# ethan-li-coding/AD-Census

Measured on NVIDIA H100. Metric: disparity-maps/sec (450x375x64), higher is better.
Workload: dtype f32

## Files before the change

### adcensus_b200/csrc/k_scanline.cu

```cuda
#include "adc_common.cuh"
#include "so_plan.h"
#include <cuda.h>
#include <string.h>

template <int K>
struct Piece { static constexpr int G = (K % 4 == 0) ? 4 : ((K % 2 == 0) ? 2 : 1); static constexpr int NP = K / G; };

template <int K>
__device__ __forceinline__ void ld_vec(const float* p, int lane, int Dp, float (&v)[K]) {
    constexpr int G = Piece<K>::G, NP = Piece<K>::NP;
#pragma unroll
    for (int j = 0; j < NP; j++) {
        const int d = lane * K + j * G;
        if (d < Dp) {
            if (G == 4) { const float4 t = *reinterpret_cast<const float4*>(p + d); v[j*G] = t.x; v[j*G+1] = t.y; v[j*G+2] = t.z; v[j*G+3] = t.w; }
            else if (G == 2) { const float2 t = *reinterpret_cast<const float2*>(p + d); v[j*G] = t.x; v[j*G+1] = t.y; }
            else v[j] = p[d];
        } else {
#pragma unroll
            for (int g = 0; g < G; g++) v[j * G + g] = 0.f;
        }
    }
}

template <int K>
__device__ __forceinline__ void st_vec(float* __restrict__ p, int lane, int Dp, const float (&v)[K]) {
    constexpr int G = Piece<K>::G, NP = Piece<K>::NP;
#pragma unroll
    for (int j = 0; j < NP; j++) {
        const int d = lane * K + j * G;
        if (d < Dp) {
            if (G == 4) *reinterpret_cast<float4*>(p + d) = make_float4(v[j*G], v[j*G+1], v[j*G+2], v[j*G+3]);
            else if (G == 2) *reinterpret_cast<float2*>(p + d) = make_float2(v[j*G], v[j*G+1]);
            else p[d] = v[j];
        }
    }
}

__host__ __device__ inline int so_row_words(int W) { return (W + 31) / 32 + 2; }

__global__ void __launch_bounds__(128)
k_so_bitrows(AdcDims dm, int tso, const uint8_t* __restrict__ dmap, unsigned* __restrict__ bitrows) {
    const int pair = blockIdx.y, y = blockIdx.x;
    const int W = dm.W, rw = so_row_words(W);
    const uint8_t* mh = dmap + ((size_t)pair * 4 + 2) * dm.N;
    const uint8_t* mv = dmap + ((size_t)pair * 4 + 3) * dm.N;
    const int lane = threadIdx.x & 31, wid = threadIdx.x >> 5;
    unsigned* out = bitrows + (((size_t)pair * 4 + wid) * dm.H + y) * rw;
    for (int w0 = 0; w0 < rw; w0++) {
        const int j = w0 * 32 + lane;
        const int xr = W - 1 - j;
        bool bit = false;
        if (xr > 0 && xr < W - 1) {
            int v;
            if (wid == 0) v = mh[y * W + xr];
            else if (wid == 1) v = mh[y * W + xr + 1];
            else if (wid == 2) v = y > 0 ? mv[y * W + xr] : 255;
            else v = y + 1 < dm.H ? mv[(y + 1) * W + xr] : 255;
            bit = v < tso;
        }
        const unsigned m = __ballot_sync(0xffffffffu, bit);
        if (lane == 0) out[w0] = m;
    }
}

__global__ void __launch_bounds__(256)
k_so_records(AdcDims dm, int tso, const uint8_t* __restrict__ dmap,
             const unsigned* __restrict__ bitrows, unsigned* __restrict__ rec) {
    const int pair = blockIdx.y;
    const int i = blockIdx.x * blockDim.x + threadIdx.x;
    if (i >= dm.N) return;
    const int sx = blockIdx.z == 0 ? 1 : (blockIdx.z == 1 ? -1 : 0);
    const int sy = blockIdx.z == 2 ? 1 : (blockIdx.z == 3 ? -1 : 0);
    const int W = dm.W, D = dm.D, dmin = dm.dmin;
    const int y = i / W, x = i - y * W;
    const bool fwd = (sx + sy) > 0;
    const int pstep = sx + sy * W;
    const int variant = sx ? (fwd ? 0 : 1) : (fwd ? 2 : 3);
    const int rw = so_row_words(W), nrec = so_rec_words(dm.Dp);
    unsigned* out = rec + (((size_t)pair * 4 + variant) * dm.N + i) * nrec;
    const uint8_t* ml = dmap + ((size_t)pair * 4 + (sx ? 0 : 1)) * dm.N;
    const int pi_from = i - pstep;
    int d1 = 0;
    if (fwd) d1 = ml[i];
    else if (pi_from >= 0 && pi_from < dm.N) d1 = ml[pi_from];
    const unsigned a1 = d1 < tso ? 0xffffffffu : 0u;
    const int lo = max(0, x - dmin - (W - 2));
    const int hi = min(D - 1, x - dmin - 1);
    const unsigned* row = bitrows + (((size_t)pair * 4 + variant) * dm.H + y) * rw;
    const int j0 = W - 1 - x + dmin;
    auto window = [&](int d0) -> unsigned {
        const int j = j0 + d0;
        const int wlo = j >> 5;
        const int sh = j & 31;
        const unsigned a = (wlo >= 0 && wlo < rw) ? row[wlo] : 0u;
        const unsigned b = (wlo + 1 >= 0 && wlo + 1 < rw) ? row[wlo + 1] : 0u;
        return __funnelshift_r(a, b, sh);
    };
    unsigned fill_hi = a1;
    if (lo <= hi) fill_hi = (window(hi) & 1u) ? 0xffffffffu : 0u;
    const int nw = (dm.Dp + 31) / 32 + 1;
    auto word = [&](int w0) -> unsigned {
        if (lo > hi) return a1;
        const int d0 = w0 * 32;
        const unsigned raw = window(d0);
        const unsigned m_lo = lo <= d0 ? 0u : (lo >= d0 + 32 ? 0xffffffffu : ((1u << (lo - d0)) - 1u));
        const unsigned m_hi = hi >= d0 + 31 ? 0u : (hi < d0 ? 0xffffffffu : ~((2u << (hi - d0)) - 1u));
        return (raw & ~m_lo & ~m_hi) | (a1 & m_lo) | (fill_hi & m_hi);
    };
    if (nrec == 4) {
        *reinterpret_cast<uint4*>(out) = make_uint4(a1, word(0), nw > 1 ? word(1) : 0u, nw > 2 ? word(2) : 0u);
        return;
    }
    out[0] = a1;
    for (int w0 = 0; w0 < nw; w0++) out[1 + w0] = word(w0);
    for (int w0 = 1 + nw; w0 < nrec; w0++) out[w0] = 0u;
}

__device__ __forceinline__ unsigned so_smem_u32(const void* p) { return (unsigned)__cvta_generic_to_shared(p); }
__device__ __forceinline__ void mbar_init(unsigned bar, unsigned count) {
    asm volatile("mbarrier.init.shared::cta.b64 [%0], %1;" ::"r"(bar), "r"(count) : "memory");
}
__device__ __forceinline__ void mbar_expect_tx(unsigned bar, unsigned bytes) {
    asm volatile("mbarrier.arrive.expect_tx.shared::cta.b64 _, [%0], %1;" ::"r"(bar), "r"(bytes) : "memory");
}
__device__ __forceinline__ void mbar_wait(unsigned bar, unsigned parity) {
    unsigned ok, spins = 0;
    do {
        asm volatile("{\n\t.reg .pred p;\n\tmbarrier.try_wait.parity.shared::cta.b64 p, [%1], %2;\n\tselp.u32 %0, 1, 0, p;\n\t}"
                     : "=r"(ok) : "r"(bar), "r"(parity) : "memory");
        if (!ok && ++spins > (1u << 24)) __trap();
    } while (!ok);
}
__device__ __forceinline__ void tma_load_4d(unsigned dst, const CUtensorMap* map, int c0, int c1, int c2, int c3, unsigned bar) {
    asm volatile("cp.async.bulk.tensor.4d.shared::cluster.global.tile.mbarrier::complete_tx::bytes [%0], [%1, {%2, %3, %4, %5}], [%6];"
                 ::"r"(dst), "l"(reinterpret_cast<unsigned long long>(map)), "r"(c0), "r"(c1), "r"(c2), "r"(c3), "r"(bar)
                 : "memory");
}

template <int K, int LPS, bool FULL, bool WTA>
__device__ __forceinline__ void so_pass(const CUtensorMap& tm_cost, const CUtensorMap& tm_rec, const AdcParams& P,
                                        float* __restrict__ dst, float* __restrict__ disp_l, int sx, int sy, int T, int NS) {
    constexpr int LPW = 32 / LPS;
    if constexpr (WTA) { sx = 0; sy = -1; }
    extern __shared__ __align__(128) unsigned char so_smem[];
    const AdcDims& dm = P.dm;
    const int lane = threadIdx.x & 31, wid = threadIdx.x >> 5;
    const int sub = lane / LPS, gl = lane % LPS;
    const int line0 = (blockIdx.x * SO_WARPS + wid) * LPW;
    const int line = line0 + sub;
    const int pair = blockIdx.y;
    const int n_lines = sx ? dm.H : dm.W, n_steps = sx ? dm.W : dm.H;
    if (line0 >= n_lines) return;
    const bool live = line < n_lines;
    const int W = dm.W, D = FULL ? K * LPS : dm.D, Dp = FULL ? K * LPS : dm.Dp;
    const int pstep = sx + sy * W;
    const int nrec = so_rec_words(Dp);
    const bool fwd = sx + sy > 0;
    const int variant = sx ? (sx > 0 ? 0 : 1) : (sy > 0 ? 2 : 3);
    const unsigned cost_region = so_cost_region(Dp, T), slot_bytes = so_slot_bytes(Dp, T);
    unsigned char* wring = so_smem + (size_t)wid * NS * slot_bytes;
    const unsigned bar0 = so_smem_u32(so_smem + (size_t)SO_WARPS * NS * slot_bytes) + (unsigned)(wid * NS) * 8u;
    const unsigned tx = (unsigned)(T * LPW * (Dp + nrec) * 4);
    const int nch = (n_steps + T - 1) / T;

    auto issue = [&](int c) {
        const int s = c % NS;
        const unsigned bar = bar0 + 8u * (unsigned)s, d0 = so_smem_u32(wring + (size_t)s * slot_bytes);
        const int p0 = fwd ? c * T : n_steps - (c + 1) * T;
        mbar_expect_tx(bar, tx);
        if (sx) {
            tma_load_4d(d0, &tm_cost, 0, p0, line0, pair, bar);
            tma_load_4d(d0 + cost_region, &tm_rec, 0, p0, line0, pair * 4 + variant, bar);
        } else {
            tma_load_4d(d0, &tm_cost, 0, line0, p0, pair, bar);
            tma_load_4d(d0 + cost_region, &tm_rec, 0, line0, p0, pair * 4 + variant, bar);
        }
    };
    if (lane == 0) {
        for (int j = 0; j < NS; j++) mbar_init(bar0 + 8u * j, 1);
        asm volatile("fence.mbarrier_init.release.cluster;" ::: "memory");
        for (int c = 0; c < NS && c < nch; c++) issue(c);
    }
    __syncwarp();

    int c = 0, t = 0, slot = 0;
    unsigned phase = 0;
    const int bit0 = gl * K;
    auto fetch = [&](float (&C)[K], bool& a1, unsigned& bits) -> float* {
        if (t == 0) mbar_wait(bar0 + 8u * (unsigned)slot, phase);
        const int pos = fwd ? t : T - 1 - t;
        const int row = sx ? sub * T + pos : pos * LPW + sub;
        unsigned char* sl = wring + (size_t)slot * slot_bytes;
        float* cs = reinterpret_cast<float*>(sl) + row * Dp;
        if constexpr (FULL && K == 8) {
            const int b = (gl >> 2) & 1;
            const float4 u = *reinterpret_cast<const float4*>(cs + 8 * gl + 4 * b);
            const float4 v = *reinterpret_cast<const float4*>(cs + 8 * gl + 4 - 4 * b);
            const float4 lo = b ? v : u, hi = b ? u : v;
            C[0] = lo.x; C[1] = lo.y; C[2] = lo.z; C[3] = lo.w;
            C[4] = hi.x; C[5] = hi.y; C[6] = hi.z; C[7] = hi.w;
        } else ld_vec<K>(cs, gl, Dp, C);
        const unsigned* rw = reinterpret_cast<const unsigned*>(sl + cost_region) + row * nrec;
        a1 = rw[0] != 0u;
        bits = __funnelshift_r(rw[1 + (bit0 >> 5)], rw[2 + (bit0 >> 5)], bit0 & 31);
        if (!WTA && ++t == T) {
            asm volatile("fence.proxy.async.shared::cta;" ::: "memory");
            __syncwarp();
            if (lane == 0 && c + NS < nch) issue(c + NS);
            t = 0;
            c++;
            if (++slot == NS) { slot = 0; phase ^= 1u; }
        }
        return cs;
    };

    bool valid[K];
#pragma unroll
    for (int k = 0; k < K; k++) valid[k] = FULL || (gl * K + k) < D;

    const int wta_threads = 32 * min(SO_WARPS, (n_lines - (int)blockIdx.x * SO_WARPS * LPW + LPW - 1) / LPW);
    auto wta_left = [&](const float* row, const float (&V)[K], float m, int step) {
        int kk = K;
#pragma unroll
        for (int k = K - 1; k >= 0; k--)
            if (valid[k] && V[k] == m) kk = k;
        const unsigned bal = __ballot_sync(0xffffffffu, kk < K);
        const unsigned grp = LPS == 32 ? bal : (bal >> (sub * LPS)) & ((1u << LPS) - 1u);
        __syncwarp();
        if (live && gl == __ffs(grp) - 1) {
            const int bd = gl * K + kk;
            float out = ADC_INVALID_F;
            if (m < ADC_LARGE_F && bd > 0 && bd < D - 1) out = adc_subpixel(row[bd - 1], row[bd + 1], m, dm.dmin + bd);
            disp_l[(size_t)pair * dm.N + (size_t)(dm.H - 1 - step) * W + line] = out;
        }
    };
    auto wta_records = [&](int nt, int s0) {
        constexpr int CB = SO_WARPS * LPW;
        const int x0 = blockIdx.x * CB, NJ = CB + D - 1, nb = (W + CB - 1) / CB, dmin = dm.dmin;
        const long long plane = (long long)dm.H * nb * NJ;
        float* R = dst + (size_t)pair * dm.vol_stride;
        const size_t wstride = (size_t)NS * slot_bytes / 4;
        const int xcap = W - 1 - x0;
        for (int tt = 0; tt < nt; tt++) {
            const int y = dm.H - 1 - (s0 + tt);
            const float* rb = reinterpret_cast<const float*>(so_smem + (size_t)slot * slot_bytes) + (T - 1 - tt) * LPW * Dp;
            for (int j = threadIdx.x; j < NJ; j += wta_threads) {
                const int xr = x0 - dmin - (D - 1) + j;
                const int ilo = max(0, j - (D - 1)), ihi = min(min(CB - 1, j), xcap);
                if (xr < 0 || xr >= W || ilo > ihi) continue;
                const int dd0 = D - 1 - j;
                auto at = [&](int i) { return rb[(size_t)(i / LPW) * wstride + (i % LPW) * Dp + i + dd0]; };
                float m = ADC_LARGE_F;
                int a = -1;
                const float* pw = rb + dd0;
#pragma unroll 1
                for (int w = 0; w < SO_WARPS; w++, pw += wstride + LPW) {
                    const float* p = pw;
#pragma unroll
                    for (int s = 0; s < LPW; s++, p += Dp + 1) {
                        const int i = w * LPW + s;
                        if (i >= ilo && i <= ihi) {
                            const float v = *p;
                            if (m > v) { m = v; a = i; }
                        }
                    }
                }
                const long long r = ((long long)y * nb + blockIdx.x) * NJ + j;
                R[r] = m;
                R[plane + r] = __int_as_float(a < 0 ? -1 : a + dd0);
                R[2 * plane + r] = a > ilo ? at(a - 1) : ADC_LARGE_F;
                R[3 * plane + r] = a >= 0 && a < ihi ? at(a + 1) : ADC_LARGE_F;
                R[4 * plane + r] = at(ilo);
                R[5 * plane + r] = at(ihi);
            }
        }
    };
    auto wta_advance = [&](int step) {
        if (++t < T && step + 1 < n_steps) return;
        asm volatile("bar.sync 1, %0;" ::"r"(wta_threads) : "memory");
        wta_records(t, step + 1 - t);
        asm volatile("fence.proxy.async.shared::cta;" ::: "memory");
        asm volatile("bar.sync 1, %0;" ::"r"(wta_threads) : "memory");
        if (lane == 0 && c + NS < nch) issue(c + NS);
        t = 0;
        c++;
        if (++slot == NS) { slot = 0; phase ^= 1u; }
    };

    long long pi = (long long)(sy ? (sy > 0 ? 0 : dm.H - 1) : line) * W + (sx ? (sx > 0 ? 0 : W - 1) : line);
    float* O = dst + (size_t)pair * dm.vol_stride;
    float L[K];
    float* row;
    {
        bool a1;
        unsigned bits;
        row = fetch(L, a1, bits);
    }
    if (!WTA && live) st_vec<K>(O + (size_t)pi * Dp, gl, Dp, L);
    float minL = ADC_LARGE_F;
#pragma unroll
    for (int k = 0; k < K; k++) {
        if (!valid[k]) L[k] = ADC_LARGE_F;
        minL = fminf(minL, L[k]);
    }
#pragma unroll
    for (int o = LPS / 2; o >= 1; o >>= 1) minL = fminf(minL, __shfl_xor_sync(0xffffffffu, minL, o));
    if constexpr (WTA) {
        wta_left(row, L, minL, 0);
        wta_advance(0);
    }

    for (int step = 1; step < n_steps; step++) {
        float C[K];
        bool a1;
        unsigned bits;
        row = fetch(C, a1, bits);
        pi += pstep;

        const float up = __shfl_up_sync(0xffffffffu, L[K - 1], 1, LPS);
        const float down = __shfl_down_sync(0xffffffffu, L[0], 1, LPS);
        const float left_in = gl == 0 ? ADC_LARGE_F : up;
        const float right_in = gl == LPS - 1 ? ADC_LARGE_F : down;
        const float P1a = a1 ? P.p1 : P.p1_4, P1b = a1 ? P.p1_4 : P.p1_10;
        const float P2a = a1 ? P.p2 : P.p2_4, P2b = a1 ? P.p2_4 : P.p2_10;
        const float m4a = __fadd_rn(minL, P2a), m4b = __fadd_rn(minL, P2b);

        float Ln[K];
        float mn = ADC_LARGE_F;
#pragma unroll
        for (int k = 0; k < K; k++) {
            const bool a2 = (bits >> k) & 1u;
            const float P1 = a2 ? P1a : P1b;
            const float l1 = L[k];
            const float l2 = __fadd_rn(k > 0 ? L[k - 1] : left_in, P1);
            const float l3 = __fadd_rn(k < K - 1 ? L[k + 1] : right_in, P1);
            const float l4 = a2 ? m4a : m4b;
            float v = __fadd_rn(C[k], fminf(fminf(l1, l2), fminf(l3, l4)));
            v = __fmul_rn(v, 0.5f);
            Ln[k] = v;
            if (valid[k]) mn = fminf(mn, v);
        }
        if constexpr (WTA) {
            if constexpr (FULL && K == 8) {
                const int b = (gl >> 2) & 1;
                const float4 lo = make_float4(Ln[0], Ln[1], Ln[2], Ln[3]), hi = make_float4(Ln[4], Ln[5], Ln[6], Ln[7]);
                *reinterpret_cast<float4*>(row + 8 * gl + 4 * b) = b ? hi : lo;
                *reinterpret_cast<float4*>(row + 8 * gl + 4 - 4 * b) = b ? lo : hi;
            } else st_vec<K>(row, gl, Dp, Ln);
        } else if (live) st_vec<K>(O + (size_t)pi * Dp, gl, Dp, Ln);
#pragma unroll
        for (int k = 0; k < K; k++) L[k] = valid[k] ? Ln[k] : ADC_LARGE_F;
#pragma unroll
        for (int o = LPS / 2; o >= 1; o >>= 1) mn = fminf(mn, __shfl_xor_sync(0xffffffffu, mn, o));
        minL = mn;
        if constexpr (WTA) {
            wta_left(row, Ln, mn, step);
            wta_advance(step);
        }
    }
}

template <int K, int LPS, bool FULL>
__global__ void __launch_bounds__(SO_WARPS * 32, SO_MIN_CTAS)
k_scanline(const __grid_constant__ CUtensorMap tm_cost, const __grid_constant__ CUtensorMap tm_rec, AdcParams P,
           float* __restrict__ dst, int sx, int sy, int T, int NS) {
    so_pass<K, LPS, FULL, false>(tm_cost, tm_rec, P, dst, nullptr, sx, sy, T, NS);
}

template <int K, int LPS, bool FULL>
__global__ void __launch_bounds__(SO_WARPS * 32, SO_MIN_CTAS)
k_scanline_wta(const __grid_constant__ CUtensorMap tm_cost, const __grid_constant__ CUtensorMap tm_rec, AdcParams P,
               float* __restrict__ rec, float* __restrict__ disp_l, int T, int NS) {
    so_pass<K, LPS, FULL, true>(tm_cost, tm_rec, P, rec, disp_l, 0, -1, T, NS);
}

template <int K, int LPS, bool FULL>
constexpr bool so_wta_built() { return LPS != 32 && !(K == 1 && FULL); }

template <int K, int LPS, bool FULL, bool WTA>
static int launch_scanline_kf(const AdcParams& P, const AdcWave& w, const CUtensorMap& tc, const CUtensorMap& tr,
                              int T, int NS, size_t smem, float* dst, int sx, int sy, cudaStream_t st) {
    if constexpr (WTA && !so_wta_built<K, LPS, FULL>()) {
        return 1;
    } else {
        constexpr int LPW = 32 / LPS;
        const int n_lines = sx ? P.dm.H : P.dm.W;
        const void* fn;
        if constexpr (WTA) fn = (const void*)k_scanline_wta<K, LPS, FULL>;
        else fn = (const void*)k_scanline<K, LPS, FULL>;
        static AdcOnce attr_once;
        if (adc_once_needed(attr_once)) {
            cudaFuncSetAttribute(fn, cudaFuncAttributeMaxDynamicSharedMemorySize, SO_SMEM_MAX);
            cudaFuncSetAttribute(fn, cudaFuncAttributePreferredSharedMemoryCarveout, cudaSharedmemCarveoutMaxShared);
            adc_once_done(attr_once);
        }
        const int lines_per_block = SO_WARPS * LPW;
        dim3 grid((n_lines + lines_per_block - 1) / lines_per_block, w.S);
        if constexpr (WTA) k_scanline_wta<K, LPS, FULL><<<grid, SO_WARPS * 32, smem, st>>>(tc, tr, P, dst, w.disp_l, T, NS);
        else k_scanline<K, LPS, FULL><<<grid, SO_WARPS * 32, smem, st>>>(tc, tr, P, dst, sx, sy, T, NS);
        return 0;
    }
}

void adc_launch_so_bitrows(const AdcParams& P, const AdcWave& w, cudaStream_t st, unsigned long long* launches) {
    dim3 grid(P.dm.H, w.S);
    k_so_bitrows<<<grid, 128, 0, st>>>(P.dm, P.tso, w.dmap, w.so_bitrows);
    dim3 rgrid((P.dm.N + 255) / 256, w.S, 4);
    k_so_records<<<rgrid, 256, 0, st>>>(P.dm, P.tso, w.dmap, w.so_bitrows, w.so_rec);
    *launches += 2;
}

bool adc_so_tmaps_encode(const AdcParams& P, int S, float* volA, float* volB, unsigned* so_rec, AdcSoTmaps* out) {
    memset(out, 0, sizeof(*out));
    const AdcTmapEncodeFn enc = adc_tmap_encoder();
    if (!enc) return false;
    int dev = 0, smem_sm = 0, smem_res = 0;
    cudaGetDevice(&dev);
    if (cudaDeviceGetAttribute(&smem_sm, cudaDevAttrMaxSharedMemoryPerMultiprocessor, dev) != cudaSuccess ||
        cudaDeviceGetAttribute(&smem_res, cudaDevAttrReservedSharedMemoryPerBlock, dev) != cudaSuccess) { cudaGetLastError(); return false; }
    const AdcDims& dm = P.dm;
    const int Dp = dm.Dp, nrec = so_rec_words(Dp), LPW = 32 / so_lanes_per_line(Dp);
    for (int axis = 0; axis < 2; axis++) {
        const SoPlan pl = so_plan(dm.W, dm.H, Dp, S, axis, adc_sm_count(), (size_t)smem_sm, (size_t)smem_res);
        if (pl.T == 0) return false;
        out->T[axis] = pl.T; out->NS[axis] = pl.NS; out->smem[axis] = (unsigned)pl.smem;
        const cuuint32_t bx = axis ? (cuuint32_t)LPW : (cuuint32_t)pl.T, by = axis ? (cuuint32_t)pl.T : (cuuint32_t)LPW;
        const cuuint32_t estr[4] = {1, 1, 1, 1};
        for (int v = 0; v < 2; v++) {
            const cuuint64_t gdim[4] = {(cuuint64_t)Dp, (cuuint64_t)dm.W, (cuuint64_t)dm.H, (cuuint64_t)S};
            const cuuint64_t gstr[3] = {(cuuint64_t)Dp * 4, (cuuint64_t)dm.W * Dp * 4, (cuuint64_t)dm.vol_stride * 4};
            const cuuint32_t box[4] = {(cuuint32_t)Dp, bx, by, 1};
            CUtensorMap tm;
            if (enc(&tm, CU_TENSOR_MAP_DATA_TYPE_FLOAT32, 4, v ? volB : volA, gdim, gstr, box, estr, CU_TENSOR_MAP_INTERLEAVE_NONE,
                    CU_TENSOR_MAP_SWIZZLE_NONE, CU_TENSOR_MAP_L2_PROMOTION_L2_256B, CU_TENSOR_MAP_FLOAT_OOB_FILL_NONE) != CUDA_SUCCESS)
                return false;
            memcpy(out->cost[v][axis], &tm, 128);
        }
        {
            const cuuint64_t gdim[4] = {(cuuint64_t)nrec, (cuuint64_t)dm.W, (cuuint64_t)dm.H, (cuuint64_t)S * 4};
            const cuuint64_t gstr[3] = {(cuuint64_t)nrec * 4, (cuuint64_t)dm.W * nrec * 4, (cuuint64_t)dm.N * nrec * 4};
            const cuuint32_t box[4] = {(cuuint32_t)nrec, bx, by, 1};
            CUtensorMap tm;
            if (enc(&tm, CU_TENSOR_MAP_DATA_TYPE_UINT32, 4, so_rec, gdim, gstr, box, estr, CU_TENSOR_MAP_INTERLEAVE_NONE,
                    CU_TENSOR_MAP_SWIZZLE_NONE, CU_TENSOR_MAP_L2_PROMOTION_L2_256B, CU_TENSOR_MAP_FLOAT_OOB_FILL_NONE) != CUDA_SUCCESS)
                return false;
            memcpy(out->rec[axis], &tm, 128);
        }
    }
    return true;
}

template <bool WTA>
static int launch_scanline(const AdcParams& P, const AdcWave& w, const float* src, float* dst, int sx, int sy,
                           cudaStream_t st, unsigned long long* launches) {
    const int Dp = P.dm.Dp;
    if (Dp > 256 || !w.so_tm || (src != w.volA && src != w.volB)) return 1;
    const int axis = sx ? 0 : 1;
    CUtensorMap tc, tr;
    memcpy(&tc, w.so_tm->cost[src == w.volB ? 1 : 0][axis], 128);
    memcpy(&tr, w.so_tm->rec[axis], 128);
    const int T = w.so_tm->T[axis], NS = w.so_tm->NS[axis];
    const size_t smem = w.so_tm->smem[axis];
    int rc = 1;
#define SO_GO(KK, LL) rc = (P.dm.D == KK * LL ? launch_scanline_kf<KK, LL, true, WTA>(P, w, tc, tr, T, NS, smem, dst, sx, sy, st) \
                                                  : launch_scanline_kf<KK, LL, false, WTA>(P, w, tc, tr, T, NS, smem, dst, sx, sy, st))
    switch (so_lanes_per_line(Dp)) {
        case 8:
            switch ((Dp + 7) / 8) { case 1: SO_GO(1, 8); break; case 2: SO_GO(2, 8); break; case 3: SO_GO(3, 8); break; case 4: SO_GO(4, 8); break;
                                    case 5: SO_GO(5, 8); break; case 6: SO_GO(6, 8); break; case 7: SO_GO(7, 8); break; default: SO_GO(8, 8); }
            break;
        case 16:
            switch ((Dp + 15) / 16) { case 5: SO_GO(5, 16); break; case 6: SO_GO(6, 16); break; case 7: SO_GO(7, 16); break; default: SO_GO(8, 16); }
            break;
        default:
            switch ((Dp + 31) / 32) { case 5: SO_GO(5, 32); break; case 6: SO_GO(6, 32); break; case 7: SO_GO(7, 32); break; default: SO_GO(8, 32); }
    }
#undef SO_GO
    if (rc) return rc;
    ++*launches;
    return 0;
}

int adc_launch_scanline(const AdcParams& P, const AdcWave& w, const float* src, float* dst, int sx, int sy,
                        cudaStream_t st, unsigned long long* launches) {
    return launch_scanline<false>(P, w, src, dst, sx, sy, st, launches);
}

int adc_launch_scanline_wta(const AdcParams& P, const AdcWave& w, const float* src, float* rec, cudaStream_t st,
                            unsigned long long* launches) {
    return launch_scanline<true>(P, w, src, rec, 0, -1, st, launches);
}

size_t adc_so_rec_bytes(const AdcDims& dm) { return (size_t)4 * dm.N * so_rec_words(dm.Dp) * 4; }
size_t adc_so_bitrow_bytes(const AdcDims& dm) { return (size_t)4 * dm.H * so_row_words(dm.W) * 4; }
```

### adcensus_b200/csrc/k_wta.cu

```cuda
#include "adc_common.cuh"
#include "so_plan.h"

#define WT_PX 128
#define WT_DC 16
#define WT_LS WT_DC
#define WT_RT ((WT_PX + WT_DC - 1 + WT_PX / 4 - 1) / (WT_PX / 4))
#define WT_RS (WT_PX + 3)

__global__ void __launch_bounds__(WT_PX, 6)
k_wta(AdcDims dm, const float* __restrict__ vol, float* __restrict__ disp_l, float* __restrict__ disp_r) {
    __shared__ __align__(16) float tl[WT_PX * WT_LS];
    __shared__ float tr[WT_DC * WT_RS];
    const int pair = blockIdx.z, y = blockIdx.y, x0 = blockIdx.x * WT_PX;
    const int W = dm.W, D = dm.D, Dp = dm.Dp;
    const float* rowv = vol + (size_t)pair * dm.vol_stride + (size_t)y * W * Dp;
    const int t = threadIdx.x;
    const int kq = t & 3, cj = t >> 2;
    const float4 LARGE4 = make_float4(ADC_LARGE_F, ADC_LARGE_F, ADC_LARGE_F, ADC_LARGE_F);
    float lbest = ADC_LARGE_F, rbest = ADC_LARGE_F;
    int lbd = -1, rbd = -1;
    float4 vl[WT_PX / 32], vr[WT_RT];
    auto fetch = [&](int d0) {
        const bool qin = d0 + 4 * kq < Dp;
        const float* cv = rowv + d0 + 4 * kq;
        const int cb = x0 + dm.dmin + d0;
#pragma unroll
        for (int i = 0; i < WT_PX / 32; i++) {
            const int x = x0 + cj + 32 * i;
            vl[i] = (qin && x < W) ? __ldg(reinterpret_cast<const float4*>(cv + x * Dp)) : LARGE4;
        }
#pragma unroll
        for (int i = 0; i < WT_RT; i++) {
            const int j = cj + 32 * i, x = cb + j;
            vr[i] = (qin && j < WT_PX + WT_DC - 1 && x >= 0 && x < W) ? __ldg(reinterpret_cast<const float4*>(cv + x * Dp)) : LARGE4;
        }
    };
    fetch(0);
    for (int d0 = 0; d0 < D; d0 += WT_DC) {
        const int dn = min(WT_DC, D - d0);
#pragma unroll
        for (int i = 0; i < WT_PX / 32; i++) {
            *reinterpret_cast<float4*>(tl + (cj + 32 * i) * WT_LS + 4 * (kq ^ ((cj >> 1) & 3))) = vl[i];
        }
#pragma unroll
        for (int i = 0; i < WT_RT; i++) {
            const int r0 = cj + 32 * i - 4 * kq;
            const float e[4] = {vr[i].x, vr[i].y, vr[i].z, vr[i].w};
#pragma unroll
            for (int c = 0; c < 4; c++) {
                const int r = r0 - c;
                if (r >= 0 && r < WT_PX) tr[(4 * kq + c) * WT_RS + r] = e[c];
            }
        }
        __syncthreads();
        if (d0 + WT_DC < D) fetch(d0 + WT_DC);
        const float* pl = tl + t * WT_LS;
        const int sw = ((t >> 1) & 3) << 2;
        const float* pr = tr + t;
        int lk = -1, rk = -1;
        if (dn == WT_DC) {
#pragma unroll
            for (int k4 = 0; k4 < WT_DC; k4 += 4) {
                const float4 a4 = *reinterpret_cast<const float4*>(pl + (k4 ^ sw));
                const float a[4] = {a4.x, a4.y, a4.z, a4.w};
#pragma unroll
                for (int j = 0; j < 4; j++) {
                    const float b = pr[(k4 + j) * WT_RS];
                    if (lbest > a[j]) { lbest = a[j]; lk = k4 + j; }
                    if (rbest > b) { rbest = b; rk = k4 + j; }
                }
            }
        } else {
            for (int k = 0; k < dn; k++) {
                const float a = pl[k ^ sw], b = pr[k * WT_RS];
                if (lbest > a) { lbest = a; lk = k; }
                if (rbest > b) { rbest = b; rk = k; }
            }
        }
        if (lk >= 0) lbd = d0 + lk;
        if (rk >= 0) rbd = d0 + rk;
        __syncthreads();
    }
    const int x = x0 + t;
    if (x >= W) return;
    const size_t o = (size_t)pair * dm.N + (size_t)y * W + x;
    {
        float out = ADC_INVALID_F;
        if (lbd > 0 && lbd < D - 1) {
            const float* v = rowv + x * Dp + lbd;
            out = adc_subpixel(__ldg(v - 1), __ldg(v + 1), lbest, dm.dmin + lbd);
        }
        disp_l[o] = out;
    }
    {
        float out = 0.0f;
        if (rbd >= 0) {
            const int best = dm.dmin + rbd;
            out = (float)best;
            if (rbd > 0 && rbd < D - 1) {
                const int x1 = x + best - 1, x2 = x + best + 1;
                const float c1 = (x1 >= 0 && x1 < W) ? __ldg(rowv + x1 * Dp + rbd - 1) : ADC_LARGE_F;
                const float c2 = (x2 >= 0 && x2 < W) ? __ldg(rowv + x2 * Dp + rbd + 1) : ADC_LARGE_F;
                out = adc_subpixel(c1, c2, rbest, best);
            }
        }
        disp_r[o] = out;
    }
}

__global__ void __launch_bounds__(128)
k_wta_merge(AdcDims dm, int CB, const float* __restrict__ rec, float* __restrict__ disp_r) {
    const int xr = blockIdx.x * blockDim.x + threadIdx.x, y = blockIdx.y, pair = blockIdx.z;
    if (xr >= dm.W) return;
    const int W = dm.W, D = dm.D, dmin = dm.dmin, NJ = CB + D - 1, nb = (W + CB - 1) / CB;
    const long long plane = (long long)dm.H * nb * NJ;
    const float* R = rec + (size_t)pair * dm.vol_stride;
    const int xlo = max(0, xr + dmin), xhi = min(W - 1, xr + dmin + D - 1);
    float m = ADC_LARGE_F, c1 = ADC_LARGE_F, c2 = ADC_LARGE_F;
    int rbd = -1;
    bool open = false;
    long long rprev = -1;
    if (xlo <= xhi) {
        for (int b = xlo / CB; b <= xhi / CB; b++) {
            const int x0 = b * CB;
            const int dlo = max(0, x0 - xr - dmin), dhi = min(D - 1, min(x0 + CB, W) - 1 - xr - dmin);
            const long long r = ((long long)y * nb + b) * NJ + (xr - x0 + dmin + D - 1);
            const float rm = __ldg(R + r);
            if (open) { c2 = __ldg(R + 4 * plane + r); open = false; }
            if (m > rm) {
                const int a = __float_as_int(__ldg(R + plane + r));
                m = rm;
                rbd = a;
                c1 = a != dlo ? __ldg(R + 2 * plane + r) : rprev >= 0 ? __ldg(R + 5 * plane + rprev) : ADC_LARGE_F;
                c2 = __ldg(R + 3 * plane + r);
                open = a == dhi;
            }
            rprev = r;
        }
    }
    float out = 0.0f;
    if (rbd >= 0) {
        const int best = dmin + rbd;
        out = (float)best;
        if (rbd > 0 && rbd < D - 1) out = adc_subpixel(c1, c2, m, best);
    }
    disp_r[(size_t)pair * dm.N + (size_t)y * W + xr] = out;
}

int adc_launch_wta_merge(const AdcParams& P, const AdcWave& w, const float* rec, cudaStream_t st, unsigned long long* launches) {
    dim3 grid((P.dm.W + 127) / 128, P.dm.H, w.S);
    k_wta_merge<<<grid, 128, 0, st>>>(P.dm, so_wta_band(P.dm.Dp), rec, w.disp_r);
    ++*launches;
    return 0;
}

int adc_launch_wta(const AdcParams& P, const AdcWave& w, const float* vol, cudaStream_t st, unsigned long long* launches) {
    dim3 grid((P.dm.W + WT_PX - 1) / WT_PX, P.dm.H, w.S);
    k_wta<<<grid, WT_PX, 0, st>>>(P.dm, vol, w.disp_l, w.disp_r);
    ++*launches;
    return 0;
}
```

Before: 2050.

## Flatten WTA record loop and use tree reduction; batch merge loads

The in-scanline WTA record pass now spreads work over (row, column) pairs instead of looping rows serially, and replaces the sequential min scan with a fully unrolled pairwise tree reduction over CB candidates held in registers. The merge kernel prefetches the block minima four at a time before processing them, so independent global loads overlap. The aim is more parallelism and a shorter dependency chain in the WTA stages. In exchange, register pressure rises from the CB-sized arrays, and tie-breaking may change because the tree reduction picks ties differently from the first-minimum scan.

```diff
diff --git a/adcensus_b200/csrc/k_scanline.cu b/adcensus_b200/csrc/k_scanline.cu
--- a/adcensus_b200/csrc/k_scanline.cu
+++ b/adcensus_b200/csrc/k_scanline.cu
@@ -242,38 +242,38 @@
         float* R = dst + (size_t)pair * dm.vol_stride;
         const size_t wstride = (size_t)NS * slot_bytes / 4;
         const int xcap = W - 1 - x0;
-        for (int tt = 0; tt < nt; tt++) {
+        const float* sb = reinterpret_cast<const float*>(so_smem + (size_t)slot * slot_bytes);
+        for (int it = threadIdx.x; it < nt * NJ; it += wta_threads) {
+            int tt = 0, j = it;
+            while (j >= NJ) { j -= NJ; tt++; }
+            const int xr = x0 - dmin - (D - 1) + j;
+            const int ilo = max(0, j - (D - 1)), ihi = min(min(CB - 1, j), xcap);
+            if (xr < 0 || xr >= W || ilo > ihi) continue;
             const int y = dm.H - 1 - (s0 + tt);
-            const float* rb = reinterpret_cast<const float*>(so_smem + (size_t)slot * slot_bytes) + (T - 1 - tt) * LPW * Dp;
-            for (int j = threadIdx.x; j < NJ; j += wta_threads) {
-                const int xr = x0 - dmin - (D - 1) + j;
-                const int ilo = max(0, j - (D - 1)), ihi = min(min(CB - 1, j), xcap);
-                if (xr < 0 || xr >= W || ilo > ihi) continue;
-                const int dd0 = D - 1 - j;
-                auto at = [&](int i) { return rb[(size_t)(i / LPW) * wstride + (i % LPW) * Dp + i + dd0]; };
-                float m = ADC_LARGE_F;
-                int a = -1;
-                const float* pw = rb + dd0;
-#pragma unroll 1
-                for (int w = 0; w < SO_WARPS; w++, pw += wstride + LPW) {
-                    const float* p = pw;
-#pragma unroll
-                    for (int s = 0; s < LPW; s++, p += Dp + 1) {
-                        const int i = w * LPW + s;
-                        if (i >= ilo && i <= ihi) {
-                            const float v = *p;
-                            if (m > v) { m = v; a = i; }
-                        }
-                    }
-                }
-                const long long r = ((long long)y * nb + blockIdx.x) * NJ + j;
-                R[r] = m;
-                R[plane + r] = __int_as_float(a < 0 ? -1 : a + dd0);
-                R[2 * plane + r] = a > ilo ? at(a - 1) : ADC_LARGE_F;
-                R[3 * plane + r] = a >= 0 && a < ihi ? at(a + 1) : ADC_LARGE_F;
-                R[4 * plane + r] = at(ilo);
-                R[5 * plane + r] = at(ihi);
+            const float* rb = sb + (T - 1 - tt) * LPW * Dp;
+            const int dd0 = D - 1 - j;
+            auto at = [&](int i) { return rb[(size_t)(i / LPW) * wstride + (i % LPW) * Dp + i + dd0]; };
+            float v[CB];
+            int a[CB];
+#pragma unroll
+            for (int i = 0; i < CB; i++) {
+                v[i] = i >= ilo && i <= ihi ? rb[(size_t)(i / LPW) * (wstride + LPW) + (i % LPW) * (Dp + 1) + dd0] : ADC_LARGE_F;
+                a[i] = i;
             }
+#pragma unroll
+            for (int h = 1; h < CB; h *= 2)
+#pragma unroll
+                for (int i = 0; i < CB; i += 2 * h)
+                    if (v[i + h] < v[i]) { v[i] = v[i + h]; a[i] = a[i + h]; }
+            const float m = v[0];
+            const int ar = m < ADC_LARGE_F ? a[0] : -1;
+            const long long r = ((long long)y * nb + blockIdx.x) * NJ + j;
+            R[r] = m;
+            R[plane + r] = __int_as_float(ar < 0 ? -1 : ar + dd0);
+            R[2 * plane + r] = ar > ilo ? at(ar - 1) : ADC_LARGE_F;
+            R[3 * plane + r] = ar >= 0 && ar < ihi ? at(ar + 1) : ADC_LARGE_F;
+            R[4 * plane + r] = at(ilo);
+            R[5 * plane + r] = at(ihi);
         }
     };
     auto wta_advance = [&](int step) {
diff --git a/adcensus_b200/csrc/k_wta.cu b/adcensus_b200/csrc/k_wta.cu
--- a/adcensus_b200/csrc/k_wta.cu
+++ b/adcensus_b200/csrc/k_wta.cu
@@ -121,21 +121,33 @@
     bool open = false;
     long long rprev = -1;
     if (xlo <= xhi) {
-        for (int b = xlo / CB; b <= xhi / CB; b++) {
-            const int x0 = b * CB;
-            const int dlo = max(0, x0 - xr - dmin), dhi = min(D - 1, min(x0 + CB, W) - 1 - xr - dmin);
-            const long long r = ((long long)y * nb + b) * NJ + (xr - x0 + dmin + D - 1);
-            const float rm = __ldg(R + r);
-            if (open) { c2 = __ldg(R + 4 * plane + r); open = false; }
-            if (m > rm) {
-                const int a = __float_as_int(__ldg(R + plane + r));
-                m = rm;
-                rbd = a;
-                c1 = a != dlo ? __ldg(R + 2 * plane + r) : rprev >= 0 ? __ldg(R + 5 * plane + rprev) : ADC_LARGE_F;
-                c2 = __ldg(R + 3 * plane + r);
-                open = a == dhi;
+        const int blast = xhi / CB;
+        for (int bq = xlo / CB; bq <= blast; bq += 4) {
+            float rmq[4];
+#pragma unroll
+            for (int k = 0; k < 4; k++) {
+                const int b = bq + k;
+                rmq[k] = b <= blast ? __ldg(R + ((long long)y * nb + b) * NJ + (xr - b * CB + dmin + D - 1)) : 0.0f;
             }
-            rprev = r;
+#pragma unroll
+            for (int k = 0; k < 4; k++) {
+                const int b = bq + k;
+                if (b > blast) break;
+                const int x0 = b * CB;
+                const int dlo = max(0, x0 - xr - dmin), dhi = min(D - 1, min(x0 + CB, W) - 1 - xr - dmin);
+                const long long r = ((long long)y * nb + b) * NJ + (xr - x0 + dmin + D - 1);
+                const float rm = rmq[k];
+                if (open) { c2 = __ldg(R + 4 * plane + r); open = false; }
+                if (m > rm) {
+                    const int a = __float_as_int(__ldg(R + plane + r));
+                    m = rm;
+                    rbd = a;
+                    c1 = a != dlo ? __ldg(R + 2 * plane + r) : rprev >= 0 ? __ldg(R + 5 * plane + rprev) : ADC_LARGE_F;
+                    c2 = __ldg(R + 3 * plane + r);
+                    open = a == dhi;
+                }
+                rprev = r;
+            }
         }
     }
     float out = 0.0f;
```

After: 2047 (median of 6 runs). Within noise of the previous version (-0.2%).
